# MengRao/pollnet

Hardware: AMD Instinct MI355X
Metric: device-resident Gbit/s + Mframes/s, 1500 B IPv4/TCP frames, 1/2/4/8 MI355X (higher is better)
Workload: dtype u16/u32 integer (one's-complement sums)

## Files before the change

### pollnet_amd/csrc/udp_demux.hpp

```cpp
#pragma once
#include <hip/hip_runtime.h>

#include "../../include/pollnet_amd.h"
#include "device_common.hpp"
#include "frame_pass.hpp"
#include "pn_internal.hpp"

namespace {

using namespace pn_dev;

constexpr uint32_t kUdHdr = 42;
constexpr uint32_t kUdMaxTiles = 1024;
constexpr uint32_t kUdMinTile = 256;
constexpr int kUdCountThreads = 256;
constexpr int kUdColThreads = 64;
constexpr int kUdScanThreads = 1024;
constexpr uint32_t kUdChunk = 4 * kWave;
constexpr int kUdBatch = 4;
constexpr uint32_t kUdSfEntries = (PN_UDP_MAX_SUBS + 1 + 3) & ~3u;
static_assert(kUdScanThreads * 4 == PN_UDP_MAX_SUBS, "the subs workgroup takes four subscriptions a thread");

struct UdArgs {
  const uint8_t* frames;
  const uint64_t* offs;
  const u32x4* results;
  uint8_t* pay;
  uint64_t cap;
  uint64_t* pay_offs;
  uint16_t* pay_lens;
  uint32_t* sub_ids;
  uint32_t* src_index;
  uint32_t* sub_first;
  uint64_t* sub_bytes;
  pn_udp_gather_total* total;
  u32x4* hdr;
  uint32_t* sf;
  uint64_t* wsum;
  uint32_t* src;
  uint32_t* hist;
  uint32_t n;
  uint32_t n_subs;
  uint32_t tile;
  uint32_t n_tiles;
  uint32_t n_chunks;
  uint32_t stride;
  uint32_t frame_off;
  uint32_t avail;
};

__device__ __forceinline__ uint32_t ud_pad16(uint32_t len) { return (len + 15u) & ~15u; }

__device__ __forceinline__ bool ud_taken(const UdArgs& a, uint32_t f, bool live, uint32_t& len, uint32_t& sub,
                                         uint64_t& src) {
  len = 0;
  sub = 0;
  src = 0;
  if (!live) return false;
  const u32x4 r = a.results[f];
  const uint32_t flags = r.w >> 16, plen = r.w & 0xffffu, poff = r.z >> 16;
  bool ok = PN_UDP_DELIVER(flags) && poff == kUdHdr && kUdHdr + plen <= a.avail && r.x < a.n_subs;
  uint64_t eth;
  if (a.offs) {
    const uint64_t o = a.offs[f];
    ok = ok && (o & 15u) == a.frame_off;
    eth = o;
  } else {
    eth = (uint64_t)f * a.stride + a.frame_off;
  }
  if (!ok) return false;
  len = plen;
  sub = r.x;
  src = (uint64_t)(uintptr_t)a.frames + eth + kUdHdr;
  return true;
}

__device__ __forceinline__ bool ud_msg(const UdArgs& a, uint32_t j, bool live, uint32_t& len, uint64_t& src) {
  uint32_t i = 0, sub;
  if (live) i = min(a.src[j], a.n - 1u);
  return ud_taken(a, i, live, len, sub, src);
}

__device__ __forceinline__ uint32_t ud_n_msgs(const UdArgs& a) {
  return min((uint32_t)__builtin_amdgcn_readfirstlane(a.hdr[0].x), a.n);
}

__device__ __forceinline__ uint32_t ud_wave_scan(uint32_t v, int lane) {
#pragma unroll
  for (int d = 1; d < kWave; d <<= 1) {
    const uint32_t t = __shfl_up(v, d);
    if (lane >= d) v += t;
  }
  return v;
}

__global__ __launch_bounds__(kUdCountThreads) void udp_demux_count_kernel(UdArgs a) {
  __shared__ uint32_t hist[PN_UDP_MAX_SUBS];
  const uint32_t t = threadIdx.x, tile = blockIdx.x;
  for (uint32_t s = t; s < a.n_subs; s += kUdCountThreads) hist[s] = 0u;
  __syncthreads();
  const uint32_t f0 = tile * a.tile, f1 = min(a.n, f0 + a.tile);
  for (uint32_t f = f0 + t; f < f1; f += kUdCountThreads) {
    uint32_t len, sub;
    uint64_t src;
    if (ud_taken(a, f, true, len, sub, src)) atomicAdd(&hist[sub], 1u);
  }
  __syncthreads();
  uint32_t* row = a.hist + (size_t)tile * a.n_subs;
  for (uint32_t s = t; s < a.n_subs; s += kUdCountThreads) row[s] = hist[s];
}

__global__ __launch_bounds__(kUdColThreads) void udp_demux_cols_kernel(UdArgs a) {
  const uint32_t s = blockIdx.x * kUdColThreads + threadIdx.x;
  if (s >= a.n_subs) return;
  uint32_t* p = a.hist + s;
  uint32_t run = 0, t = 0;
  for (; t + 8 <= a.n_tiles; t += 8) {
    uint32_t c[8];
#pragma unroll
    for (int k = 0; k < 8; ++k) c[k] = p[(size_t)(t + k) * a.n_subs];
#pragma unroll
    for (int k = 0; k < 8; ++k) {
      p[(size_t)(t + k) * a.n_subs] = run;
      run += c[k];
    }
  }
  for (; t < a.n_tiles; ++t) {
    const uint32_t c = p[(size_t)t * a.n_subs];
    p[(size_t)t * a.n_subs] = run;
    run += c;
  }
  a.sf[s] = run;
}

__global__ __launch_bounds__(kUdScanThreads) void udp_demux_subs_kernel(UdArgs a) {
  __shared__ uint32_t w_tot[kUdScanThreads / kWave];
  const int t = threadIdx.x, lane = t & (kWave - 1), wv = t / kWave;
  uint32_t v[4], sum = 0;
#pragma unroll
  for (int k = 0; k < 4; ++k) {
    const uint32_t s = 4u * t + k;
    v[k] = a.n && s < a.n_subs ? a.sf[s] : 0u;
    sum += v[k];
  }
  const uint32_t inc = ud_wave_scan(sum, lane);
  if (lane == kWave - 1) w_tot[wv] = inc;
  __syncthreads();
  uint32_t ex = inc - sum, tot = 0;
#pragma unroll
  for (int k = 0; k < kUdScanThreads / kWave; ++k) {
    if (k < wv) ex += w_tot[k];
    tot += w_tot[k];
  }
#pragma unroll
  for (int k = 0; k < 4; ++k) {
    const uint32_t s = 4u * t + k;
    if (s < a.n_subs) {
      const uint32_t first = min(ex, a.n);
      if (a.n) a.sf[s] = first;
      a.sub_first[s] = first;
      if (!a.n) a.sub_bytes[s] = 0ull;
    }
    ex += v[k];
  }
  if (t == 0) {
    tot = min(tot, a.n);
    a.sub_first[a.n_subs] = tot;
    if (a.n) {
      a.sf[a.n_subs] = tot;
      a.hdr[0] = u32x4{tot, 0u, 0u, 0u};
    } else {
      a.sub_bytes[a.n_subs] = 0ull;
      pn_udp_gather_total z;
      z.n_bytes = 0;
      z.n_msgs = 0;
      z.n_fit = 0;
      *a.total = z;
    }
  }
}

__global__ __launch_bounds__(kWave) void udp_demux_place_kernel(UdArgs a) {
  __shared__ uint32_t cur[PN_UDP_MAX_SUBS];
  const uint32_t lane = threadIdx.x, tile = blockIdx.x;
  const uint32_t* row = a.hist + (size_t)tile * a.n_subs;
  for (uint32_t s = lane; s < a.n_subs; s += kWave) cur[s] = a.sf[s] + row[s];
  __syncthreads();
  const uint32_t key_bits = 32u - (uint32_t)__builtin_clz(a.n_subs | 1u);
  const uint64_t below = (1ull << lane) - 1ull;
  const uint32_t f0 = tile * a.tile, f1 = min(a.n, f0 + a.tile);
  for (uint32_t base = f0; base < f1; base += kWave) {
    const uint32_t f = base + lane;
    uint32_t len, sub;
    uint64_t src;
    const bool taken = ud_taken(a, f, f < f1, len, sub, src);
    uint64_t peers = __ballot(taken);
    for (uint32_t b = 0; b < key_bits; ++b) {
      const bool bit = (sub >> b) & 1u;
      const uint64_t bal = __ballot(bit);
      peers &= bit ? bal : ~bal;
    }
    const uint32_t rank = (uint32_t)__popcll(peers & below), cnt = (uint32_t)__popcll(peers);
    const uint32_t c = taken ? cur[sub] : 0u;
    __syncthreads();
    if (taken && rank + 1u == cnt) cur[sub] = c + cnt;
    __syncthreads();
    if (taken) {
      const uint32_t j = min(c + rank, a.n - 1u);
      a.pay_lens[j] = (uint16_t)len;
      a.sub_ids[j] = sub;
      a.src[j] = f;
      if (a.src_index) a.src_index[j] = f;
    }
  }
}

__global__ __launch_bounds__(kWave) void udp_demux_sum_kernel(UdArgs a) {
  const uint32_t lane = threadIdx.x, chunk = blockIdx.x;
  const uint32_t n_msgs = ud_n_msgs(a);
  const uint32_t jb = chunk * kUdChunk;
  uint32_t bytes = 0;
  if (jb < n_msgs) {
#pragma unroll
    for (uint32_t p = 0; p < kUdChunk / kWave; ++p) {
      const uint32_t j = jb + p * kWave + lane;
      uint32_t len;
      uint64_t src;
      const bool taken = ud_msg(a, j, j < n_msgs, len, src);
      bytes += taken ? ud_pad16(len) : 0u;
    }
  }
  bytes = ud_wave_scan(bytes, (int)lane);
  if (lane == kWave - 1) a.wsum[chunk] = bytes;
}

__global__ __launch_bounds__(kUdScanThreads) void udp_demux_scan_kernel(UdArgs a) {
  __shared__ uint64_t w_bytes[kUdScanThreads / kWave];
  const int t = threadIdx.x, lane = t & (kWave - 1), wv = t / kWave;
  uint64_t carry = 0;
  for (uint32_t c0 = 0; c0 < a.n_chunks; c0 += kUdScanThreads) {
    const uint32_t c = c0 + t;
    const bool in = c < a.n_chunks;
    const uint32_t e = in ? (uint32_t)a.wsum[c] : 0u;
    const uint32_t ib = ud_wave_scan(e, lane);
    if (lane == kWave - 1) w_bytes[wv] = ib;
    __syncthreads();
    uint64_t bb = carry, tb = 0;
#pragma unroll
    for (int k = 0; k < kUdScanThreads / kWave; ++k) {
      if (k < wv) bb += w_bytes[k];
      tb += w_bytes[k];
    }
    if (in) a.wsum[c] = bb + ib - e;
    carry += tb;
    __syncthreads();
  }
  if (t == 0) {
    const uint32_t n_msgs = min(a.hdr[0].x, a.n);
    a.hdr[0] = u32x4{n_msgs, 0u, (uint32_t)carry, (uint32_t)(carry >> 32)};
    pn_udp_gather_total tot;
    tot.n_bytes = carry;
    tot.n_msgs = n_msgs;
    tot.n_fit = n_msgs;
    *a.total = tot;
  }
}

template <int SH>
__global__ __launch_bounds__(kWave) void udp_demux_copy_kernel(UdArgs a) {
  static_assert(SH == 0 || SH == 2, "the payload starts 0 or 2 bytes into a dword");
  const int lane = threadIdx.x;
  const uint32_t n_msgs = ud_n_msgs(a);
  const uint32_t p0 = blockIdx.x * kWave;
  if (p0 >= n_msgs) return;
  const uint32_t chunk = p0 / kUdChunk;
  const uint64_t e = a.wsum[chunk];
  uint64_t byte_base =
      ((uint64_t)__builtin_amdgcn_readfirstlane((uint32_t)(e >> 32)) << 32) | (uint32_t)__builtin_amdgcn_readfirstlane((uint32_t)e);
  for (uint32_t q0 = chunk * kUdChunk; q0 < p0; q0 += kWave) {
    uint32_t q_len;
    uint64_t q_src;
    const bool q_taken = ud_msg(a, q0 + lane, true, q_len, q_src);
    const uint32_t q_inc = ud_wave_scan(q_taken ? ud_pad16(q_len) : 0u, lane);
    byte_base += (uint32_t)__builtin_amdgcn_readlane(q_inc, kWave - 1);
  }

  auto emit = [&](uint8_t* dst, const u32x4& x, uint32_t xe, int c, int len) {
    uint32_t o[4];
    if constexpr (SH == 0) {
      o[0] = x.x, o[1] = x.y, o[2] = x.z, o[3] = x.w;
    } else {
      o[0] = __builtin_amdgcn_alignbyte(x.y, x.x, SH), o[1] = __builtin_amdgcn_alignbyte(x.z, x.y, SH);
      o[2] = __builtin_amdgcn_alignbyte(x.w, x.z, SH), o[3] = __builtin_amdgcn_alignbyte(xe, x.w, SH);
    }
#pragma unroll
    for (int q = 0; q < 4; ++q) {
      int k = len - (16 * c + 4 * q);
      k = k < 0 ? 0 : (k > 4 ? 4 : k);
      o[q] &= k >= 4 ? 0xFFFFFFFFu : ((1u << (8 * k)) - 1u);
    }
    const u32x4 v = {o[0], o[1], o[2], o[3]};
    __builtin_nontemporal_store(v, reinterpret_cast<u32x4*>(dst + 16 * c));
  };

  {
    const uint32_t cnt = min((uint32_t)kWave, n_msgs - p0);
    const uint32_t j = p0 + lane;
    const bool has = (uint32_t)lane < cnt;
    uint32_t m_len;
    uint64_t m_src;
    const bool taken = ud_msg(a, j, has, m_len, m_src);
    const uint32_t pad = ud_pad16(m_len);
    const uint32_t inc = ud_wave_scan(pad, lane);
    const uint32_t m_boff = inc - pad;
    const uint64_t off = byte_base + m_boff;
    const bool fits = has && taken && off <= a.cap && pad <= a.cap - off;
    if (has) {
      a.pay_offs[j] = off;
      if (off <= a.cap && pad > a.cap - off) a.total->n_fit = j;
    }
    const uint32_t meta = m_len | (fits ? 0x10000u : 0u);

    for (uint32_t g = 0; g < cnt; g += 8) {
      const uint32_t mi = g + ((uint32_t)lane >> 3);
      const int c = lane & 7, ml = (int)(mi & 63);
      const uint32_t meta_m = __shfl(meta, ml);
      const uint32_t b_m = __shfl(m_boff, ml);
      const uint32_t s_lo = __shfl((uint32_t)m_src, ml), s_hi = __shfl((uint32_t)(m_src >> 32), ml);
      const int len = (int)(meta_m & 0xffffu);
      if (!(mi < cnt && (meta_m & 0x10000u) && 16 * c < len)) continue;
      const uint32_t* s = reinterpret_cast<const uint32_t*>((((uint64_t)s_hi << 32) | s_lo) - SH);
      const int lim = SH + len;
      uint32_t v[5];
#pragma unroll
      for (int k = 0; k < (SH ? 5 : 4); ++k) v[k] = 4 * (4 * c + k) < lim ? s[4 * c + k] : 0u;
      if constexpr (SH == 0) v[4] = 0u;
      emit(a.pay + byte_base + b_m, u32x4{v[0], v[1], v[2], v[3]}, v[4], c, len);
    }

    uint64_t need = __ballot(fits && m_len > 128);
    while (need) {
      int lens_b[kUdBatch];
      uint8_t* dsts[kUdBatch];
      u32x4 w[kUdBatch][2];
      uint32_t we[kUdBatch][2];
      __amdgpu_buffer_rsrc_t rss[kUdBatch];
#pragma unroll
      for (int q = 0; q < kUdBatch; ++q) {
        const bool hasq = need != 0;
        const int fi = hasq ? __builtin_ctzll(need) : 0;
        if (hasq) need &= need - 1;
        const uint32_t ln = hasq ? (uint32_t)__builtin_amdgcn_readlane(m_len, fi) : 0u;
        lens_b[q] = (int)ln;
        const uint32_t s_lo = __builtin_amdgcn_readlane((uint32_t)m_src, fi);
        const uint32_t s_hi = __builtin_amdgcn_readlane((uint32_t)(m_src >> 32), fi);
        dsts[q] = a.pay + byte_base + (uint32_t)__builtin_amdgcn_readlane(m_boff, fi);
        rss[q] = frame_rsrc((const uint8_t*)((((uint64_t)s_hi << 32) | s_lo) - SH), ln ? ((SH + ln + 3) & ~3u) : 0u);
#pragma unroll
        for (int s = 0; s < 2; ++s) {
          const uint32_t vo = 128 + 16 * lane + 1024 * s;
          w[q][s] = __builtin_amdgcn_raw_buffer_load_b128(rss[q], vo, 0, 0);
          we[q][s] = SH ? __builtin_amdgcn_raw_buffer_load_b32(rss[q], vo + 16, 0, 0) : 0u;
        }
      }
      __builtin_amdgcn_sched_barrier(0);
#pragma unroll
      for (int q = 0; q < kUdBatch; ++q) {
        const int len = lens_b[q];
        if (16 * (8 + lane) < len) emit(dsts[q], w[q][0], we[q][0], 8 + lane, len);
        if (16 * (72 + lane) < len) emit(dsts[q], w[q][1], we[q][1], 72 + lane, len);
        for (int c0 = 136; 16 * c0 < len; c0 += 64) {
          const uint32_t vo = 16 * (c0 + lane);
          const u32x4 x = __builtin_amdgcn_raw_buffer_load_b128(rss[q], vo, 0, 0);
          const uint32_t xe = SH ? __builtin_amdgcn_raw_buffer_load_b32(rss[q], vo + 16, 0, 0) : 0u;
          if (16 * (c0 + lane) < len) emit(dsts[q], x, xe, c0 + lane, len);
        }
      }
    }
  }
}

__global__ __launch_bounds__(kUdCountThreads) void udp_demux_subbytes_kernel(UdArgs a) {
  const uint32_t s = blockIdx.x * kUdCountThreads + threadIdx.x;
  if (s > a.n_subs) return;
  const u32x4 h = a.hdr[0];
  const uint32_t n_msgs = min(h.x, a.n), first = a.sf[s];
  a.sub_bytes[s] = first >= n_msgs ? (((uint64_t)h.w << 32) | h.z) : a.pay_offs[first];
}


struct UdPlan {
  uint32_t tile, n_tiles, n_chunks;
  size_t off_sf, off_wsum, off_src, off_hist, bytes;
};

inline UdPlan ud_plan(uint32_t n, uint32_t n_subs) {
  UdPlan p = {};
  if (!n) return p;
  const uint32_t per = (n - 1) / kUdMaxTiles + 1;
  p.tile = per <= kUdMinTile ? kUdMinTile : (per + kWave - 1) / kWave * kWave;
  p.n_tiles = (n - 1) / p.tile + 1;
  p.n_chunks = (n - 1) / kUdChunk + 1;
  auto up16 = [](size_t b) { return (b + 15) & ~(size_t)15; };
  p.off_sf = 16;
  p.off_wsum = p.off_sf + 4 * (size_t)kUdSfEntries;
  p.off_src = p.off_wsum + up16(8 * (size_t)p.n_chunks);
  p.off_hist = p.off_src + up16(4 * (size_t)n);
  p.bytes = p.off_hist + up16(4 * (size_t)p.n_tiles * n_subs);
  return p;
}

inline int ud_scratch(pn_ctx* ctx, size_t bytes, hipStream_t s) {
  if (bytes > ctx->ud_scratch_bytes) {
    if (ctx->ud_scratch) {
      const int rc = pn_internal::fence_host_wait(ctx, ctx->ud);
      if (rc) return rc;
      (void)hipFree(ctx->ud_scratch);
      ctx->ud_scratch = nullptr;
      ctx->ud_scratch_bytes = 0;
    }
    const size_t cap = bytes < ((size_t)1 << 20) ? ((size_t)1 << 20) : bytes;
    hipError_t e = hipMalloc(&ctx->ud_scratch, cap);
    if (e != hipSuccess) return pn_internal::hip_err(ctx, e, "hipMalloc(udp demux scratch)");
    ctx->ud_scratch_bytes = cap;
  }
  return pn_internal::fence_use(ctx, ctx->ud, s);
}

inline int ud_launch(pn_ctx* ctx, UdArgs& a, hipStream_t s) {
  const UdPlan p = ud_plan(a.n, a.n_subs);
  a.tile = p.tile;
  a.n_tiles = p.n_tiles;
  a.n_chunks = p.n_chunks;
  if (a.n) {
    const int rc = ud_scratch(ctx, p.bytes, s);
    if (rc) return rc;
    uint8_t* b = (uint8_t*)ctx->ud_scratch;
    a.hdr = (u32x4*)b;
    a.sf = (uint32_t*)(b + p.off_sf);
    a.wsum = (uint64_t*)(b + p.off_wsum);
    a.src = (uint32_t*)(b + p.off_src);
    a.hist = (uint32_t*)(b + p.off_hist);
    hipLaunchKernelGGL(udp_demux_count_kernel, dim3(a.n_tiles), dim3(kUdCountThreads), 0, s, a);
    hipLaunchKernelGGL(udp_demux_cols_kernel, dim3((a.n_subs - 1) / kUdColThreads + 1), dim3(kUdColThreads), 0, s, a);
  }
  hipLaunchKernelGGL(udp_demux_subs_kernel, dim3(1), dim3(kUdScanThreads), 0, s, a);
  if (a.n) {
    hipLaunchKernelGGL(udp_demux_place_kernel, dim3(a.n_tiles), dim3(kWave), 0, s, a);
    hipLaunchKernelGGL(udp_demux_sum_kernel, dim3(a.n_chunks), dim3(kWave), 0, s, a);
    hipLaunchKernelGGL(udp_demux_scan_kernel, dim3(1), dim3(kUdScanThreads), 0, s, a);
    if ((a.frame_off + kUdHdr) & 2) hipLaunchKernelGGL(udp_demux_copy_kernel<2>, dim3((a.n - 1) / kWave + 1), dim3(kWave), 0, s, a);
    else hipLaunchKernelGGL(udp_demux_copy_kernel<0>, dim3((a.n - 1) / kWave + 1), dim3(kWave), 0, s, a);
    hipLaunchKernelGGL(udp_demux_subbytes_kernel, dim3(a.n_subs / kUdCountThreads + 1), dim3(kUdCountThreads), 0, s, a);
  }
  const hipError_t e = hipGetLastError();
  if (e != hipSuccess) return pn_internal::hip_err(ctx, e, "udp_demux launch");
  pn_internal::note_stream(ctx, s);
  return PN_OK;
}

}
```

### pollnet_amd/csrc/udp_gather.hpp

```cpp
#pragma once
#include <hip/hip_runtime.h>

#include "../../include/pollnet_amd.h"
#include "device_common.hpp"
#include "frame_pass.hpp"
#include "pn_internal.hpp"

namespace {

using namespace pn_dev;

constexpr uint32_t kUgHdr = 42;
constexpr int kUgScanThreads = 1024;
constexpr int kUgBatch = 4;

struct UgArgs {
  const uint8_t* frames;
  const uint64_t* offs;
  const u32x4* results;
  uint8_t* pay;
  uint64_t cap;
  uint64_t* pay_offs;
  uint16_t* pay_lens;
  uint32_t* sub_ids;
  uint32_t* src_index;
  u32x4* scratch;
  pn_udp_gather_total* total;
  uint32_t n;
  uint32_t n_waves;
  uint32_t stride;
  uint32_t frame_off;
  uint32_t avail;
  uint32_t fpw;
};

__device__ __forceinline__ uint32_t ug_pad16(uint32_t len) { return (len + 15u) & ~15u; }

__device__ __forceinline__ bool ug_taken(const UgArgs& a, uint32_t f, bool live, uint32_t& len, uint32_t& sub,
                                         uint64_t& src) {
  len = 0;
  sub = 0;
  src = 0;
  if (!live) return false;
  const u32x4 r = a.results[f];
  const uint32_t flags = r.w >> 16, plen = r.w & 0xffffu, poff = r.z >> 16;
  bool ok = PN_UDP_DELIVER(flags) && poff == kUgHdr && kUgHdr + plen <= a.avail;
  uint64_t eth;
  if (a.offs) {
    const uint64_t o = a.offs[f];
    ok = ok && (o & 15u) == a.frame_off;
    eth = o;
  } else {
    eth = (uint64_t)f * a.stride + a.frame_off;
  }
  if (!ok) return false;
  len = plen;
  sub = r.x;
  src = (uint64_t)(uintptr_t)a.frames + eth + kUgHdr;
  return true;
}

__device__ __forceinline__ uint32_t ug_wave_scan(uint32_t v, int lane) {
#pragma unroll
  for (int d = 1; d < kWave; d <<= 1) {
    const uint32_t t = __shfl_up(v, d);
    if (lane >= d) v += t;
  }
  return v;
}

__device__ __forceinline__ uint32_t ug_wave_sum(uint32_t v) {
  v += dpp<0xB1>(v);
  v += dpp<0x4E>(v);
  v += dpp<0x141>(v);
  v += dpp<0x128>(v);
  return __builtin_amdgcn_readlane(v, 0) + __builtin_amdgcn_readlane(v, 16) + __builtin_amdgcn_readlane(v, 32) +
         __builtin_amdgcn_readlane(v, 48);
}

struct UgMsg {
  uint32_t cnt;
  uint32_t len, sub, boff, sl;
  uint64_t src;
};

__device__ __forceinline__ UgMsg ug_compact(bool taken, uint32_t len, uint32_t sub, uint64_t src, int lane) {
  UgMsg m;
  const uint64_t tk = __ballot(taken);
  m.cnt = (uint32_t)__popcll(tk);
  const uint32_t rank = (uint32_t)__popcll(tk & ((1ull << lane) - 1ull));
  const uint32_t dest = taken ? rank : m.cnt + ((uint32_t)lane - rank);
  m.sl = (uint32_t)__builtin_amdgcn_ds_permute((int)(dest * 4), lane);
  const bool has = (uint32_t)lane < m.cnt;
  const uint32_t len_r = __shfl(len, m.sl);
  m.len = has ? len_r : 0u;
  m.sub = __shfl(sub, m.sl);
  const uint32_t lo = __shfl((uint32_t)src, m.sl), hi = __shfl((uint32_t)(src >> 32), m.sl);
  m.src = has ? (((uint64_t)hi << 32) | lo) : 0ull;
  const uint32_t pad = ug_pad16(m.len);
  m.boff = ug_wave_scan(pad, lane) - pad;
  return m;
}

__global__ __launch_bounds__(kWave) void udp_gather_count_kernel(UgArgs a) {
  const int lane = threadIdx.x;
  const uint32_t group = xcd_group(blockIdx.x, gridDim.x);
  const uint32_t wave_base = group * a.fpw;
  if (wave_base >= a.n) return;
  const uint32_t n_here = min(a.fpw, a.n - wave_base);
  uint32_t len, sub;
  uint64_t src;
  const bool taken = ug_taken(a, wave_base + lane, (uint32_t)lane < n_here, len, sub, src);
  const uint32_t msgs = (uint32_t)__popcll(__ballot(taken));
  const uint32_t bytes = ug_wave_sum(taken ? ug_pad16(len) : 0u);
  if (lane == 0) a.scratch[group] = u32x4{msgs, bytes, 0u, 0u};
}

__global__ __launch_bounds__(kUgScanThreads) void udp_gather_scan_kernel(UgArgs a) {
  __shared__ uint32_t w_msgs[kUgScanThreads / kWave];
  __shared__ uint64_t w_bytes[kUgScanThreads / kWave];
  __shared__ uint32_t cross_wave, cross_msgs;
  __shared__ uint64_t cross_bytes;
  const int t = threadIdx.x, lane = t & (kWave - 1), wv = t / kWave;
  if (t == 0) cross_wave = 0xFFFFFFFFu;
  __syncthreads();
  uint32_t carry_m = 0;
  uint64_t carry_b = 0;
  for (uint32_t w0 = 0; w0 < a.n_waves; w0 += kUgScanThreads) {
    const uint32_t w = w0 + t;
    const bool in = w < a.n_waves;
    u32x4 e = {0u, 0u, 0u, 0u};
    if (in) e = a.scratch[w];
    const uint32_t im = ug_wave_scan(e.x, lane);
    const uint32_t ib = ug_wave_scan(e.y, lane);
    if (lane == kWave - 1) {
      w_msgs[wv] = im;
      w_bytes[wv] = ib;
    }
    __syncthreads();
    uint32_t bm = carry_m, tm = 0;
    uint64_t bb = carry_b, tb = 0;
#pragma unroll
    for (int k = 0; k < kUgScanThreads / kWave; ++k) {
      if (k < wv) {
        bm += w_msgs[k];
        bb += w_bytes[k];
      }
      tm += w_msgs[k];
      tb += w_bytes[k];
    }
    const uint32_t ex_m = bm + im - e.x;
    const uint64_t ex_b = bb + ib - e.y;
    if (in) {
      a.scratch[w] = u32x4{ex_m, 0u, (uint32_t)ex_b, (uint32_t)(ex_b >> 32)};
      if (ex_b <= a.cap && ex_b + e.y > a.cap) {
        cross_wave = w;
        cross_msgs = ex_m;
        cross_bytes = ex_b;
      }
    }
    carry_m += tm;
    carry_b += tb;
    __syncthreads();
  }
  if (wv != 0) return;
  uint32_t n_fit = carry_m;
  const uint32_t cw = cross_wave;
  if (cw != 0xFFFFFFFFu) {
    const uint32_t wave_base = cw * a.fpw;
    const uint32_t n_here = wave_base < a.n ? min(a.fpw, a.n - wave_base) : 0u;
    uint32_t len, sub;
    uint64_t src;
    const bool taken = ug_taken(a, wave_base + lane, (uint32_t)lane < n_here, len, sub, src);
    const uint32_t pad = taken ? ug_pad16(len) : 0u;
    const uint32_t end = ug_wave_scan(pad, lane);
    n_fit = cross_msgs + (uint32_t)__popcll(__ballot(taken && cross_bytes + end <= a.cap));
  }
  if (lane == 0) {
    pn_udp_gather_total tot;
    tot.n_bytes = carry_b;
    tot.n_msgs = carry_m;
    tot.n_fit = n_fit;
    *a.total = tot;
  }
}

template <int SH>
__global__ __launch_bounds__(kWave) void udp_gather_copy_kernel(UgArgs a) {
  static_assert(SH == 0 || SH == 2, "the payload starts 0 or 2 bytes into a dword");
  const int lane = threadIdx.x;
  const uint32_t group = xcd_group(blockIdx.x, gridDim.x);
  const uint32_t wave_base = group * a.fpw;
  if (wave_base >= a.n) return;
  const uint32_t n_here = min(a.fpw, a.n - wave_base);

  uint32_t len0, sub0;
  uint64_t src0;
  const bool taken = ug_taken(a, wave_base + lane, (uint32_t)lane < n_here, len0, sub0, src0);
  const UgMsg m = ug_compact(taken, len0, sub0, src0, lane);
  if (m.cnt == 0) return;
  const u32x4 e = a.scratch[group];
  const uint32_t e_m = __builtin_amdgcn_readfirstlane(e.x);
  const uint32_t msg_base = min(e_m, wave_base);
  const uint64_t byte_base =
      ((uint64_t)__builtin_amdgcn_readfirstlane(e.w) << 32) | (uint32_t)__builtin_amdgcn_readfirstlane(e.z);
  const bool has = (uint32_t)lane < m.cnt;
  const uint64_t off = byte_base + m.boff;
  const uint32_t pad = ug_pad16(m.len);
  const bool fits = has && off <= a.cap && pad <= a.cap - off;
  if (has) {
    const uint32_t j = msg_base + lane;
    a.pay_offs[j] = off;
    a.pay_lens[j] = (uint16_t)m.len;
    a.sub_ids[j] = m.sub;
    if (a.src_index) a.src_index[j] = wave_base + m.sl;
  }
  const uint32_t meta = m.len | (fits ? 0x10000u : 0u);

  auto emit = [&](uint8_t* dst, const u32x4& x, uint32_t xe, int c, int len) {
    uint32_t o[4];
    if constexpr (SH == 0) {
      o[0] = x.x, o[1] = x.y, o[2] = x.z, o[3] = x.w;
    } else {
      o[0] = __builtin_amdgcn_alignbyte(x.y, x.x, SH), o[1] = __builtin_amdgcn_alignbyte(x.z, x.y, SH);
      o[2] = __builtin_amdgcn_alignbyte(x.w, x.z, SH), o[3] = __builtin_amdgcn_alignbyte(xe, x.w, SH);
    }
#pragma unroll
    for (int q = 0; q < 4; ++q) {
      int k = len - (16 * c + 4 * q);
      k = k < 0 ? 0 : (k > 4 ? 4 : k);
      o[q] &= k >= 4 ? 0xFFFFFFFFu : ((1u << (8 * k)) - 1u);
    }
    const u32x4 v = {o[0], o[1], o[2], o[3]};
    __builtin_nontemporal_store(v, reinterpret_cast<u32x4*>(dst + 16 * c));
  };

  for (uint32_t g = 0; g < m.cnt; g += 8) {
    const uint32_t mi = g + ((uint32_t)lane >> 3);
    const int c = lane & 7, ml = (int)(mi & 63);
    const uint32_t meta_m = __shfl(meta, ml);
    const uint32_t b_m = __shfl(m.boff, ml);
    const uint32_t s_lo = __shfl((uint32_t)m.src, ml), s_hi = __shfl((uint32_t)(m.src >> 32), ml);
    const int len = (int)(meta_m & 0xffffu);
    if (!(mi < m.cnt && (meta_m & 0x10000u) && 16 * c < len)) continue;
    const uint32_t* s = reinterpret_cast<const uint32_t*>((((uint64_t)s_hi << 32) | s_lo) - SH);
    const int lim = SH + len;
    uint32_t v[5];
#pragma unroll
    for (int k = 0; k < (SH ? 5 : 4); ++k) v[k] = 4 * (4 * c + k) < lim ? s[4 * c + k] : 0u;
    if constexpr (SH == 0) v[4] = 0u;
    emit(a.pay + byte_base + b_m, u32x4{v[0], v[1], v[2], v[3]}, v[4], c, len);
  }

  uint64_t need = __ballot(fits && m.len > 128);
  while (need) {
    int lens_b[kUgBatch];
    uint8_t* dsts[kUgBatch];
    u32x4 w[kUgBatch][2];
    uint32_t we[kUgBatch][2];
    __amdgpu_buffer_rsrc_t rss[kUgBatch];
#pragma unroll
    for (int j = 0; j < kUgBatch; ++j) {
      const bool hasj = need != 0;
      const int fi = hasj ? __builtin_ctzll(need) : 0;
      if (hasj) need &= need - 1;
      const uint32_t ln = hasj ? (uint32_t)__builtin_amdgcn_readlane(m.len, fi) : 0u;
      lens_b[j] = (int)ln;
      const uint32_t s_lo = __builtin_amdgcn_readlane((uint32_t)m.src, fi);
      const uint32_t s_hi = __builtin_amdgcn_readlane((uint32_t)(m.src >> 32), fi);
      dsts[j] = a.pay + byte_base + (uint32_t)__builtin_amdgcn_readlane(m.boff, fi);
      rss[j] = frame_rsrc((const uint8_t*)((((uint64_t)s_hi << 32) | s_lo) - SH), ln ? ((SH + ln + 3) & ~3u) : 0u);
#pragma unroll
      for (int s = 0; s < 2; ++s) {
        const uint32_t vo = 128 + 16 * lane + 1024 * s;
        w[j][s] = __builtin_amdgcn_raw_buffer_load_b128(rss[j], vo, 0, 0);
        we[j][s] = SH ? __builtin_amdgcn_raw_buffer_load_b32(rss[j], vo + 16, 0, 0) : 0u;
      }
    }
    __builtin_amdgcn_sched_barrier(0);
#pragma unroll
    for (int j = 0; j < kUgBatch; ++j) {
      const int len = lens_b[j];
      if (16 * (8 + lane) < len) emit(dsts[j], w[j][0], we[j][0], 8 + lane, len);
      if (16 * (72 + lane) < len) emit(dsts[j], w[j][1], we[j][1], 72 + lane, len);
      for (int c0 = 136; 16 * c0 < len; c0 += 64) {
        const uint32_t vo = 16 * (c0 + lane);
        const u32x4 x = __builtin_amdgcn_raw_buffer_load_b128(rss[j], vo, 0, 0);
        const uint32_t xe = SH ? __builtin_amdgcn_raw_buffer_load_b32(rss[j], vo + 16, 0, 0) : 0u;
        if (16 * (c0 + lane) < len) emit(dsts[j], x, xe, c0 + lane, len);
      }
    }
  }
}


inline int ug_scratch(pn_ctx* ctx, uint32_t n_waves, hipStream_t s) {
  if (n_waves > ctx->ug_scratch_n) {
    if (ctx->ug_scratch) {
      const int rc = pn_internal::fence_host_wait(ctx, ctx->ug);
      if (rc) return rc;
      (void)hipFree(ctx->ug_scratch);
      ctx->ug_scratch = nullptr;
      ctx->ug_scratch_n = 0;
    }
    const uint32_t cap = n_waves < (1u << 14) ? (1u << 14) : n_waves;
    hipError_t e = hipMalloc(&ctx->ug_scratch, (size_t)cap * sizeof(u32x4));
    if (e != hipSuccess) return pn_internal::hip_err(ctx, e, "hipMalloc(udp gather scratch)");
    ctx->ug_scratch_n = cap;
  }
  return pn_internal::fence_use(ctx, ctx->ug, s);
}

inline int ug_launch(pn_ctx* ctx, UgArgs& a, hipStream_t s) {
  a.fpw = frames_per_wave(a.n);
  a.n_waves = a.n ? (a.n - 1) / a.fpw + 1 : 0;
  a.scratch = nullptr;
  if (a.n) {
    const int rc = ug_scratch(ctx, a.n_waves, s);
    if (rc) return rc;
    a.scratch = (u32x4*)ctx->ug_scratch;
    hipLaunchKernelGGL(udp_gather_count_kernel, dim3(a.n_waves), dim3(kWave), 0, s, a);
  }
  hipLaunchKernelGGL(udp_gather_scan_kernel, dim3(1), dim3(kUgScanThreads), 0, s, a);
  if (a.n) {
    if ((a.frame_off + kUgHdr) & 2) hipLaunchKernelGGL(udp_gather_copy_kernel<2>, dim3(a.n_waves), dim3(kWave), 0, s, a);
    else hipLaunchKernelGGL(udp_gather_copy_kernel<0>, dim3(a.n_waves), dim3(kWave), 0, s, a);
  }
  const hipError_t e = hipGetLastError();
  if (e != hipSuccess) return pn_internal::hip_err(ctx, e, "udp_gather launch");
  pn_internal::note_stream(ctx, s);
  return PN_OK;
}

}
```

Measured before the change: 51130.

## Parallelize demux column scan by segments and batch loads in place and gather scan

Splits the per-subscription column prefix over tiles into two phases: segments of 32 tiles are scanned in parallel, then the segment totals are scanned, and the place kernel adds the segment base. The place kernel now issues eight waves of result loads ahead before the ballot ranking, and the sum kernel stores per-quarter prefixes so the gather no longer rescans earlier quarters. The gather scan processes 16 entries per lane with DPP scans and buffer loads and stores. These changes add an extra kernel launch, more scratch memory and higher register pressure.

```diff
diff --git a/pollnet_amd/csrc/udp_demux.hpp b/pollnet_amd/csrc/udp_demux.hpp
--- a/pollnet_amd/csrc/udp_demux.hpp
+++ b/pollnet_amd/csrc/udp_demux.hpp
@@ -15,10 +15,13 @@
 constexpr uint32_t kUdMinTile = 256;
 constexpr int kUdCountThreads = 256;
 constexpr int kUdColThreads = 64;
+constexpr uint32_t kUdSeg = 32;
+constexpr int kUdAhead = 8;
 constexpr int kUdScanThreads = 1024;
 constexpr uint32_t kUdChunk = 4 * kWave;
 constexpr int kUdBatch = 4;
 constexpr uint32_t kUdSfEntries = (PN_UDP_MAX_SUBS + 1 + 3) & ~3u;
+static_assert(kUdChunk == 4 * kWave, "the sum stores one prefix per quarter of a chunk: four to a u32x4");
 static_assert(kUdScanThreads * 4 == PN_UDP_MAX_SUBS, "the subs workgroup takes four subscriptions a thread");
 
 struct UdArgs {
@@ -37,12 +40,16 @@
   u32x4* hdr;
   uint32_t* sf;
   uint64_t* wsum;
+  u32x4* qsum;
   uint32_t* src;
   uint32_t* hist;
+  uint32_t* seg;
   uint32_t n;
   uint32_t n_subs;
   uint32_t tile;
   uint32_t n_tiles;
+  uint32_t n_segs;
+  uint32_t phase;
   uint32_t n_chunks;
   uint32_t stride;
   uint32_t frame_off;
@@ -51,18 +58,24 @@
 
 __device__ __forceinline__ uint32_t ud_pad16(uint32_t len) { return (len + 15u) & ~15u; }
 
-__device__ __forceinline__ bool ud_taken(const UdArgs& a, uint32_t f, bool live, uint32_t& len, uint32_t& sub,
-                                         uint64_t& src) {
+__device__ __forceinline__ void ud_load(const UdArgs& a, uint32_t f, bool live, u32x4& r, uint64_t& o) {
+  r = u32x4{0u, 0u, 0u, 0u};
+  o = 0;
+  if (!live) return;
+  r = a.results[f];
+  if (a.offs) o = a.offs[f];
+}
+
+__device__ __forceinline__ bool ud_test(const UdArgs& a, uint32_t f, bool live, const u32x4& r, uint64_t o,
+                                        uint32_t& len, uint32_t& sub, uint64_t& src) {
   len = 0;
   sub = 0;
   src = 0;
   if (!live) return false;
-  const u32x4 r = a.results[f];
   const uint32_t flags = r.w >> 16, plen = r.w & 0xffffu, poff = r.z >> 16;
   bool ok = PN_UDP_DELIVER(flags) && poff == kUdHdr && kUdHdr + plen <= a.avail && r.x < a.n_subs;
   uint64_t eth;
   if (a.offs) {
-    const uint64_t o = a.offs[f];
     ok = ok && (o & 15u) == a.frame_off;
     eth = o;
   } else {
@@ -75,6 +88,14 @@
   return true;
 }
 
+__device__ __forceinline__ bool ud_taken(const UdArgs& a, uint32_t f, bool live, uint32_t& len, uint32_t& sub,
+                                         uint64_t& src) {
+  u32x4 r;
+  uint64_t o;
+  ud_load(a, f, live, r, o);
+  return ud_test(a, f, live, r, o, len, sub, src);
+}
+
 __device__ __forceinline__ bool ud_msg(const UdArgs& a, uint32_t j, bool live, uint32_t& len, uint64_t& src) {
   uint32_t i = 0, sub;
   if (live) i = min(a.src[j], a.n - 1u);
@@ -92,6 +113,15 @@
     if (lane >= d) v += t;
   }
   return v;
+}
+
+__device__ __forceinline__ uint32_t ud_wave_sum(uint32_t v) {
+  v += dpp<0xB1>(v);
+  v += dpp<0x4E>(v);
+  v += dpp<0x141>(v);
+  v += dpp<0x128>(v);
+  return __builtin_amdgcn_readlane(v, 0) + __builtin_amdgcn_readlane(v, 16) + __builtin_amdgcn_readlane(v, 32) +
+         __builtin_amdgcn_readlane(v, 48);
 }
 
 __global__ __launch_bounds__(kUdCountThreads) void udp_demux_count_kernel(UdArgs a) {
@@ -110,27 +140,38 @@
   for (uint32_t s = t; s < a.n_subs; s += kUdCountThreads) row[s] = hist[s];
 }
 
+__device__ __forceinline__ uint32_t ud_col_scan(uint32_t* p, uint32_t cnt, uint32_t n_subs) {
+  uint32_t run = 0, t = 0;
+  for (; t + 8 <= cnt; t += 8) {
+    uint32_t c[8];
+#pragma unroll
+    for (int k = 0; k < 8; ++k) c[k] = p[(size_t)(t + k) * n_subs];
+#pragma unroll
+    for (int k = 0; k < 8; ++k) {
+      p[(size_t)(t + k) * n_subs] = run;
+      run += c[k];
+    }
+  }
+  for (; t < cnt; ++t) {
+    const uint32_t c = p[(size_t)t * n_subs];
+    p[(size_t)t * n_subs] = run;
+    run += c;
+  }
+  return run;
+}
+
 __global__ __launch_bounds__(kUdColThreads) void udp_demux_cols_kernel(UdArgs a) {
-  const uint32_t s = blockIdx.x * kUdColThreads + threadIdx.x;
+  const uint32_t n_blocks = (a.n_subs - 1) / kUdColThreads + 1;
+  const uint32_t s = (blockIdx.x % n_blocks) * kUdColThreads + threadIdx.x;
   if (s >= a.n_subs) return;
-  uint32_t* p = a.hist + s;
-  uint32_t run = 0, t = 0;
-  for (; t + 8 <= a.n_tiles; t += 8) {
-    uint32_t c[8];
-#pragma unroll
-    for (int k = 0; k < 8; ++k) c[k] = p[(size_t)(t + k) * a.n_subs];
-#pragma unroll
-    for (int k = 0; k < 8; ++k) {
-      p[(size_t)(t + k) * a.n_subs] = run;
-      run += c[k];
-    }
-  }
-  for (; t < a.n_tiles; ++t) {
-    const uint32_t c = p[(size_t)t * a.n_subs];
-    p[(size_t)t * a.n_subs] = run;
-    run += c;
-  }
-  a.sf[s] = run;
+  if (a.phase == 0) {
+    const uint32_t g = blockIdx.x / n_blocks;
+    if (g >= a.n_segs) return;
+    const uint32_t t0 = g * kUdSeg, cnt = min(kUdSeg, a.n_tiles - t0);
+    a.seg[(size_t)g * a.n_subs + s] = ud_col_scan(a.hist + (size_t)t0 * a.n_subs + s, cnt, a.n_subs);
+  } else {
+    a.sf[s] = ud_col_scan(a.seg + s, a.n_segs, a.n_subs);
+  }
 }
 
 __global__ __launch_bounds__(kUdScanThreads) void udp_demux_subs_kernel(UdArgs a) {
@@ -184,33 +225,58 @@
   __shared__ uint32_t cur[PN_UDP_MAX_SUBS];
   const uint32_t lane = threadIdx.x, tile = blockIdx.x;
   const uint32_t* row = a.hist + (size_t)tile * a.n_subs;
-  for (uint32_t s = lane; s < a.n_subs; s += kWave) cur[s] = a.sf[s] + row[s];
+  const uint32_t* segb = a.seg + (size_t)(tile / kUdSeg) * a.n_subs;
+  for (uint32_t s0 = 0; s0 < a.n_subs; s0 += 4 * kWave) {
+    uint32_t v[4];
+#pragma unroll
+    for (int k = 0; k < 4; ++k) {
+      const uint32_t s = min(s0 + k * kWave + lane, a.n_subs - 1u);
+      v[k] = a.sf[s] + segb[s] + row[s];
+    }
+#pragma unroll
+    for (int k = 0; k < 4; ++k) {
+      const uint32_t s = s0 + k * kWave + lane;
+      if (s < a.n_subs) cur[s] = v[k];
+    }
+  }
   __syncthreads();
   const uint32_t key_bits = 32u - (uint32_t)__builtin_clz(a.n_subs | 1u);
   const uint64_t below = (1ull << lane) - 1ull;
   const uint32_t f0 = tile * a.tile, f1 = min(a.n, f0 + a.tile);
-  for (uint32_t base = f0; base < f1; base += kWave) {
-    const uint32_t f = base + lane;
-    uint32_t len, sub;
-    uint64_t src;
-    const bool taken = ud_taken(a, f, f < f1, len, sub, src);
-    uint64_t peers = __ballot(taken);
-    for (uint32_t b = 0; b < key_bits; ++b) {
-      const bool bit = (sub >> b) & 1u;
-      const uint64_t bal = __ballot(bit);
-      peers &= bit ? bal : ~bal;
-    }
-    const uint32_t rank = (uint32_t)__popcll(peers & below), cnt = (uint32_t)__popcll(peers);
-    const uint32_t c = taken ? cur[sub] : 0u;
-    __syncthreads();
-    if (taken && rank + 1u == cnt) cur[sub] = c + cnt;
-    __syncthreads();
-    if (taken) {
-      const uint32_t j = min(c + rank, a.n - 1u);
-      a.pay_lens[j] = (uint16_t)len;
-      a.sub_ids[j] = sub;
-      a.src[j] = f;
-      if (a.src_index) a.src_index[j] = f;
+  for (uint32_t b0 = f0; b0 < f1; b0 += kUdAhead * kWave) {
+    u32x4 recs[kUdAhead];
+    uint64_t eths[kUdAhead];
+#pragma unroll
+    for (int k = 0; k < kUdAhead; ++k) {
+      const uint32_t f = b0 + k * kWave + lane;
+      ud_load(a, f, f < f1, recs[k], eths[k]);
+    }
+#pragma unroll
+    for (int k = 0; k < kUdAhead; ++k) {
+      const uint32_t base = b0 + k * kWave;
+      if (base >= f1) break;
+      const uint32_t f = base + lane;
+      uint32_t len, sub;
+      uint64_t src;
+      const bool taken = ud_test(a, f, f < f1, recs[k], eths[k], len, sub, src);
+      uint64_t peers = __ballot(taken);
+      for (uint32_t b = 0; b < key_bits; ++b) {
+        const bool bit = (sub >> b) & 1u;
+        const uint64_t bal = __ballot(bit);
+        peers &= bit ? bal : ~bal;
+      }
+      const uint32_t rank = (uint32_t)__popcll(peers & below), cnt = (uint32_t)__popcll(peers);
+      const uint32_t c = taken ? cur[sub] : 0u;
+      __syncthreads();
+      if (taken && rank + 1u == cnt) cur[sub] = c + cnt;
+      __syncthreads();
+      if (taken) {
+        const uint32_t j = min(c + rank, a.n - 1u);
+        a.pay_lens[j] = (uint16_t)len;
+        a.sub_ids[j] = sub;
+        a.src[j] = f;
+        if (a.src_index) a.src_index[j] = f;
+      }
     }
   }
 }
@@ -219,8 +285,9 @@
   const uint32_t lane = threadIdx.x, chunk = blockIdx.x;
   const uint32_t n_msgs = ud_n_msgs(a);
   const uint32_t jb = chunk * kUdChunk;
-  uint32_t bytes = 0;
+  uint32_t q[kUdChunk / kWave] = {};
   if (jb < n_msgs) {
+    uint32_t bytes = 0;
 #pragma unroll
     for (uint32_t p = 0; p < kUdChunk / kWave; ++p) {
       const uint32_t j = jb + p * kWave + lane;
@@ -228,10 +295,13 @@
       uint64_t src;
       const bool taken = ud_msg(a, j, j < n_msgs, len, src);
       bytes += taken ? ud_pad16(len) : 0u;
-    }
-  }
-  bytes = ud_wave_scan(bytes, (int)lane);
-  if (lane == kWave - 1) a.wsum[chunk] = bytes;
+      q[p] = ud_wave_sum(bytes);
+    }
+  }
+  if (lane == 0) {
+    a.wsum[chunk] = q[3];
+    a.qsum[chunk] = u32x4{q[0], q[1], q[2], q[3]};
+  }
 }
 
 __global__ __launch_bounds__(kUdScanThreads) void udp_demux_scan_kernel(UdArgs a) {
@@ -277,12 +347,10 @@
   const uint64_t e = a.wsum[chunk];
   uint64_t byte_base =
       ((uint64_t)__builtin_amdgcn_readfirstlane((uint32_t)(e >> 32)) << 32) | (uint32_t)__builtin_amdgcn_readfirstlane((uint32_t)e);
-  for (uint32_t q0 = chunk * kUdChunk; q0 < p0; q0 += kWave) {
-    uint32_t q_len;
-    uint64_t q_src;
-    const bool q_taken = ud_msg(a, q0 + lane, true, q_len, q_src);
-    const uint32_t q_inc = ud_wave_scan(q_taken ? ud_pad16(q_len) : 0u, lane);
-    byte_base += (uint32_t)__builtin_amdgcn_readlane(q_inc, kWave - 1);
+  const uint32_t quarter = blockIdx.x % (kUdChunk / kWave);
+  if (quarter) {
+    const u32x4 qs = a.qsum[chunk];
+    byte_base += (uint32_t)__builtin_amdgcn_readfirstlane(quarter == 1 ? qs.x : quarter == 2 ? qs.y : qs.z);
   }
 
   auto emit = [&](uint8_t* dst, const u32x4& x, uint32_t xe, int c, int len) {
@@ -390,8 +458,8 @@
 
 
 struct UdPlan {
-  uint32_t tile, n_tiles, n_chunks;
-  size_t off_sf, off_wsum, off_src, off_hist, bytes;
+  uint32_t tile, n_tiles, n_segs, n_chunks;
+  size_t off_sf, off_wsum, off_qsum, off_src, off_seg, off_hist, bytes;
 };
 
 inline UdPlan ud_plan(uint32_t n, uint32_t n_subs) {
@@ -400,12 +468,15 @@
   const uint32_t per = (n - 1) / kUdMaxTiles + 1;
   p.tile = per <= kUdMinTile ? kUdMinTile : (per + kWave - 1) / kWave * kWave;
   p.n_tiles = (n - 1) / p.tile + 1;
+  p.n_segs = (p.n_tiles - 1) / kUdSeg + 1;
   p.n_chunks = (n - 1) / kUdChunk + 1;
   auto up16 = [](size_t b) { return (b + 15) & ~(size_t)15; };
   p.off_sf = 16;
   p.off_wsum = p.off_sf + 4 * (size_t)kUdSfEntries;
-  p.off_src = p.off_wsum + up16(8 * (size_t)p.n_chunks);
-  p.off_hist = p.off_src + up16(4 * (size_t)n);
+  p.off_qsum = p.off_wsum + up16(8 * (size_t)p.n_chunks);
+  p.off_src = p.off_qsum + 16 * (size_t)p.n_chunks;
+  p.off_seg = p.off_src + up16(4 * (size_t)n);
+  p.off_hist = p.off_seg + up16(4 * (size_t)p.n_segs * n_subs);
   p.bytes = p.off_hist + up16(4 * (size_t)p.n_tiles * n_subs);
   return p;
 }
@@ -431,6 +502,7 @@
   const UdPlan p = ud_plan(a.n, a.n_subs);
   a.tile = p.tile;
   a.n_tiles = p.n_tiles;
+  a.n_segs = p.n_segs;
   a.n_chunks = p.n_chunks;
   if (a.n) {
     const int rc = ud_scratch(ctx, p.bytes, s);
@@ -439,10 +511,16 @@
     a.hdr = (u32x4*)b;
     a.sf = (uint32_t*)(b + p.off_sf);
     a.wsum = (uint64_t*)(b + p.off_wsum);
+    a.qsum = (u32x4*)(b + p.off_qsum);
     a.src = (uint32_t*)(b + p.off_src);
+    a.seg = (uint32_t*)(b + p.off_seg);
     a.hist = (uint32_t*)(b + p.off_hist);
     hipLaunchKernelGGL(udp_demux_count_kernel, dim3(a.n_tiles), dim3(kUdCountThreads), 0, s, a);
-    hipLaunchKernelGGL(udp_demux_cols_kernel, dim3((a.n_subs - 1) / kUdColThreads + 1), dim3(kUdColThreads), 0, s, a);
+    const uint32_t col_blocks = (a.n_subs - 1) / kUdColThreads + 1;
+    a.phase = 0;
+    hipLaunchKernelGGL(udp_demux_cols_kernel, dim3(col_blocks * a.n_segs), dim3(kUdColThreads), 0, s, a);
+    a.phase = 1;
+    hipLaunchKernelGGL(udp_demux_cols_kernel, dim3(col_blocks), dim3(kUdColThreads), 0, s, a);
   }
   hipLaunchKernelGGL(udp_demux_subs_kernel, dim3(1), dim3(kUdScanThreads), 0, s, a);
   if (a.n) {
diff --git a/pollnet_amd/csrc/udp_gather.hpp b/pollnet_amd/csrc/udp_gather.hpp
--- a/pollnet_amd/csrc/udp_gather.hpp
+++ b/pollnet_amd/csrc/udp_gather.hpp
@@ -12,6 +12,7 @@
 
 constexpr uint32_t kUgHdr = 42;
 constexpr int kUgScanThreads = 1024;
+constexpr int kUgScanK = 16;
 constexpr int kUgBatch = 4;
 
 struct UgArgs {
@@ -69,6 +70,20 @@
   return v;
 }
 
+template <int CTRL, int ROWS>
+__device__ __forceinline__ uint32_t ug_dpp0(uint32_t v) {
+  return (uint32_t)__builtin_amdgcn_update_dpp(0, (int)v, CTRL, ROWS, 0xf, false);
+}
+__device__ __forceinline__ uint32_t ug_wave_scan_dpp(uint32_t v) {
+  v += ug_dpp0<0x111, 0xf>(v);
+  v += ug_dpp0<0x112, 0xf>(v);
+  v += ug_dpp0<0x114, 0xf>(v);
+  v += ug_dpp0<0x118, 0xf>(v);
+  v += ug_dpp0<0x142, 0xa>(v);
+  v += ug_dpp0<0x143, 0xc>(v);
+  return v;
+}
+
 __device__ __forceinline__ uint32_t ug_wave_sum(uint32_t v) {
   v += dpp<0xB1>(v);
   v += dpp<0x4E>(v);
@@ -126,37 +141,63 @@
   __syncthreads();
   uint32_t carry_m = 0;
   uint64_t carry_b = 0;
-  for (uint32_t w0 = 0; w0 < a.n_waves; w0 += kUgScanThreads) {
-    const uint32_t w = w0 + t;
-    const bool in = w < a.n_waves;
-    u32x4 e = {0u, 0u, 0u, 0u};
-    if (in) e = a.scratch[w];
-    const uint32_t im = ug_wave_scan(e.x, lane);
-    const uint32_t ib = ug_wave_scan(e.y, lane);
-    if (lane == kWave - 1) {
-      w_msgs[wv] = im;
-      w_bytes[wv] = ib;
+  const __amdgpu_buffer_rsrc_t rs = frame_rsrc((const uint8_t*)a.scratch, a.n_waves * 16u);
+  for (uint32_t w0 = 0; w0 < a.n_waves; w0 += kUgScanThreads * kUgScanK) {
+    const uint32_t wr = w0 + (uint32_t)wv * (kWave * kUgScanK) + (uint32_t)lane;
+    uint2 e[kUgScanK];
+#pragma unroll
+    for (int k = 0; k < kUgScanK; ++k) {
+      const auto v = __builtin_amdgcn_raw_buffer_load_b64(rs, (wr + k * kWave) * 16u, 0, 0);
+      e[k] = uint2{v[0], v[1]};
+    }
+    static_assert((uint64_t)(kWave * kUgScanK - 1) << 22 < (1ull << 32), "xb: the bytes before an entry of the wave, in 32 bits");
+    uint32_t xm[kUgScanK], xb[kUgScanK], wm = 0;
+    uint64_t wb = 0;
+    __builtin_amdgcn_sched_barrier(0);
+#pragma unroll
+    for (int k = 0; k < kUgScanK; ++k) {
+      const uint32_t im = ug_wave_scan_dpp(e[k].x), ib = ug_wave_scan_dpp(e[k].y);
+      xm[k] = wm + im - e[k].x;
+      xb[k] = (uint32_t)wb + ib - e[k].y;
+      asm volatile("" : "+v"(xm[k]), "+v"(xb[k]));
+      wm += (uint32_t)__builtin_amdgcn_readlane(im, kWave - 1);
+      wb += (uint32_t)__builtin_amdgcn_readlane(ib, kWave - 1);
+    }
+    if (lane == 0) {
+      w_msgs[wv] = wm;
+      w_bytes[wv] = wb;
     }
     __syncthreads();
+    const int wl = lane & (kUgScanThreads / kWave - 1);
+    const uint32_t vm = w_msgs[wl];
+    const uint64_t vb = w_bytes[wl];
+    const int wu = __builtin_amdgcn_readfirstlane(wv);
     uint32_t bm = carry_m, tm = 0;
     uint64_t bb = carry_b, tb = 0;
 #pragma unroll
     for (int k = 0; k < kUgScanThreads / kWave; ++k) {
-      if (k < wv) {
-        bm += w_msgs[k];
-        bb += w_bytes[k];
+      const uint32_t m = __builtin_amdgcn_readlane(vm, k);
+      const uint64_t b = ((uint64_t)(uint32_t)__builtin_amdgcn_readlane((uint32_t)(vb >> 32), k) << 32) |
+                         (uint32_t)__builtin_amdgcn_readlane((uint32_t)vb, k);
+      if (k < wu) {
+        bm += m;
+        bb += b;
       }
-      tm += w_msgs[k];
-      tb += w_bytes[k];
-    }
-    const uint32_t ex_m = bm + im - e.x;
-    const uint64_t ex_b = bb + ib - e.y;
-    if (in) {
-      a.scratch[w] = u32x4{ex_m, 0u, (uint32_t)ex_b, (uint32_t)(ex_b >> 32)};
-      if (ex_b <= a.cap && ex_b + e.y > a.cap) {
-        cross_wave = w;
-        cross_msgs = ex_m;
-        cross_bytes = ex_b;
+      tm += m;
+      tb += b;
+    }
+#pragma unroll
+    for (int k = 0; k < kUgScanK; ++k) {
+      const uint32_t w = wr + k * kWave;
+      const uint32_t ex_m = bm + xm[k];
+      const uint64_t ex_b = bb + xb[k];
+      if (w < a.n_waves) {
+        __builtin_amdgcn_raw_buffer_store_b128(u32x4{ex_m, 0u, (uint32_t)ex_b, (uint32_t)(ex_b >> 32)}, rs, w * 16u, 0, 0);
+        if (ex_b <= a.cap && ex_b + e[k].y > a.cap) {
+          cross_wave = w;
+          cross_msgs = ex_m;
+          cross_bytes = ex_b;
+        }
       }
     }
     carry_m += tm;
```

After: 51120 (median of 2 runs). No clear change (-0.0%).
